# JasonHopeSpace/panda

Measured on AMD Instinct MI355X. Metric: MSM points/s (BN254, 2^24), higher is better.
Workload: dtype u32; 1 GPU; BN254 MSM 2^24 points per GPU, Jacobian output, bases and scalars resident in HBM; curve=bn254, log_points_per_gpu=24, exchange=none

## Files before the change

panda_amd/csrc/fe29.h:

```cpp
#pragma once
#include <stdint.h>

#include "fe29_params.h"

#if defined(__HIPCC__)
#define PANDA_HD __host__ __device__ inline __attribute__((always_inline))
#else
#define PANDA_HD inline __attribute__((always_inline))
#endif

#if defined(FE29_CHECK)
#include <assert.h>
#define FE29_SHADOW_DECL unsigned __int128 shadow = 0;
#define FE29_SHADOW_MAC(x, y) shadow += (unsigned __int128)(x) * (y);
#define FE29_SHADOW_SHIFT()                                      \
    assert(shadow < ((unsigned __int128)1 << 64) && "fe29 column accumulator overflow"); \
    shadow >>= 29;
#else
#define FE29_SHADOW_DECL
#define FE29_SHADOW_MAC(x, y)
#define FE29_SHADOW_SHIFT()
#endif

#if defined(__HIP_DEVICE_COMPILE__) && !defined(FE29_NO_ASM)
// ... 359 lines not shown
    Fe<F> t;
    fe_add_nr(t, a, b);
    fe_norm(r, t);
}

template <class F>
struct SubMargin {
    static constexpr int value = (F::P[F::N - 1] >= 16) ? 1 : 6;
};

template <class F, int KB>
PANDA_HD void fe_sub(Fe<F> &r, const Fe<F> &a, const Fe<F> &b)
{
    if constexpr (IsExt2<F>::value) {
        fe_sub<typename F::Base, KB>(ext_c0(r), ext_c0(a), ext_c0(b));
        fe_sub<typename F::Base, KB>(ext_c1(r), ext_c1(a), ext_c1(b));
        return;
    } else {
    constexpr int K = KB + SubMargin<F>::value;
    static_assert(K <= 200, "subtraction constant table too small");
    Fe<F> t;
#pragma unroll
    for (int i = 0; i < F::N; i++) {
#if defined(FE29_CHECK)
        assert((u64)a.l[i] + F::KP[K][i] >= b.l[i] && (u64)a.l[i] + F::KP[K][i] - b.l[i] < (1ull << 32) && "fe_sub limb range");
#endif
        t.l[i] = a.l[i] + F::KP[K][i] - b.l[i];
    }
    fe_norm(r, t);
    }
}

template <class F, int K>
PANDA_HD constexpr u32 fe_kp30(int i)
{
    return i == 0 ? F::KP[K][0] - (2u << LIMB_BITS) : (i < F::N - 1 ? F::KP[K][i] - (2u << LIMB_BITS) + 2u : F::KP[K][i] + 2u);
}

template <class F>
struct RawOperandOk {
    static constexpr bool value = F::N <= 9;
};

template <class F, int KB>
PANDA_HD void fe_sub_raw(Fe<F> &r, const Fe<F> &a, const Fe<F> &b)
{
    static_assert(RawOperandOk<F>::value, "no column headroom for a raw operand in this field");
    constexpr int K = KB + SubMargin<F>::value;
    static_assert(K <= 200, "subtraction constant table too small");
#pragma unroll
    for (int i = 0; i < F::N; i++) {
        const u32 kp = fe_kp30<F, K>(i);
#if defined(FE29_CHECK)
        assert((u64)a.l[i] + kp >= b.l[i] && (u64)a.l[i] + kp - b.l[i] < (1ull << 31) + (1ull << 24) && "fe_sub_raw limb range");
#endif
        r.l[i] = a.l[i] + kp - b.l[i];
    }
}

template <class F, int K, int U>
PANDA_HD constexpr u32 fe_kp_bias(int i)
{
    static_assert(U >= 2 && U <= 4, "bias in units of 2^29");
    return i == 0 ? F::KP[K][0] - ((u32)(4 - U) << LIMB_BITS) : (i < F::N - 1 ? F::KP[K][i] - ((u32)(4 - U) << LIMB_BITS) + (u32)(4 - U) : F::KP[K][i] + (u32)(4 - U));
}
template <class F, int KB, int U>
PANDA_HD void fe_sub_raw_bias(Fe<F> &r, const Fe<F> &a, const Fe<F> &b)
{
    static_assert(RawOperandOk<F>::value, "no column headroom for a raw operand in this field");
    constexpr int K = KB + SubMargin<F>::value;
    static_assert(K <= 200, "subtraction constant table too small");
#pragma unroll
    for (int i = 0; i < F::N; i++) {
        const u32 kp = fe_kp_bias<F, K, U>(i);
#if defined(FE29_CHECK)
        assert((u64)a.l[i] + kp >= b.l[i] && (u64)a.l[i] + kp - b.l[i] < 3 * (1ull << 30) + 64 && "fe_sub_raw_bias limb range");
#endif
        r.l[i] = a.l[i] + kp - b.l[i];
    }
}

template <class F, int KB>
PANDA_HD void fe_neg_raw(Fe<F> &r, const Fe<F> &a)
{
    static_assert(RawOperandOk<F>::value, "no column headroom for a raw operand in this field");
    constexpr int K = KB + SubMargin<F>::value;
#pragma unroll
    for (int i = 0; i < F::N; i++) {
        const u32 kp = fe_kp30<F, K>(i);
#if defined(FE29_CHECK)
        assert(kp >= a.l[i] && "fe_neg_raw limb range");
#endif
        r.l[i] = kp - a.l[i];
    }
}

template <class F, int KB>
struct SubGrowth {
    static constexpr int value = F::KEFF[KB + SubMargin<F>::value];
};

template <class F, int KB>
PANDA_HD void fe_neg(Fe<F> &r, const Fe<F> &a)
{
    if constexpr (IsExt2<F>::value) {
        fe_neg<typename F::Base, KB>(ext_c0(r), ext_c0(a));
        fe_neg<typename F::Base, KB>(ext_c1(r), ext_c1(a));
        return;
    } else {
    constexpr int K = KB + SubMargin<F>::value;
    Fe<F> t;
#pragma unroll
    for (int i = 0; i < F::N; i++) {
#if defined(FE29_CHECK)
        assert(F::KP[K][i] >= a.l[i] && "fe_neg limb range");
#endif
        t.l[i] = F::KP[K][i] - a.l[i];
    }
    fe_norm(r, t);
    }
}

template <class F>
PANDA_HD void fe_unpack(Fe<F> &r, const u32 *w)
{
    constexpr int N = F::N, L = F::L;
#pragma unroll
    for (int k = 0; k < N; k++) {
        const int bit = 29 * k, wi = bit >> 5, sh = bit & 31;
        u32 v = 0;
        if (wi < L) {
            v = w[wi] >> sh;
            if (sh > 3 && wi + 1 < L) v |= w[wi + 1] << (32 - sh);
        }
        r.l[k] = (k < N - 1) ? (v & LIMB_MASK) : v;
    }
}

template <class F>
PANDA_HD void fe_pack(u32 *w, const Fe<F> &a)
{
    constexpr int N = F::N, L = F::L;
#pragma unroll
    for (int i = 0; i < L; i++) {
        const int bit = 32 * i, j = bit / 29, s = bit - 29 * j;
        u32 v = a.l[j] >> s;
        if (j + 1 < N) v |= a.l[j + 1] << (29 - s);
        if (29 - s + 29 < 32 && j + 2 < N) v |= a.l[j + 2] << (58 - s);
        w[i] = v;
    }
}

template <class F>
PANDA_HD void fe_carry(Fe<F> &a)
{
#pragma unroll
    for (int i = 0; i < F::N - 1; i++) {
#if defined(FE29_CHECK)
        assert((u64)a.l[i + 1] + (a.l[i] >> LIMB_BITS) < (1ull << 32) && "fe_carry limb range");
#endif
        a.l[i + 1] += a.l[i] >> LIMB_BITS;
        a.l[i] &= LIMB_MASK;
    }
}

template <class F>
PANDA_HD void fe_reduce_once(Fe<F> &a)
{
    constexpr int N = F::N;
    u32 d[N];
    u32 borrow = 0;
#pragma unroll
    for (int i = 0; i < N; i++) {
        u32 t = a.l[i] - F::P[i] - borrow;
        borrow = t >> 31;
        d[i] = (i < N - 1) ? (t & LIMB_MASK) : t;
    }
#pragma unroll
    for (int i = 0; i < N; i++) a.l[i] = borrow ? a.l[i] : d[i];
}

template <class F>
PANDA_HD void fe_reduce_small_2p(Fe<F> &a)
{
    constexpr int N = F::N;
    fe_carry(a);
    u32 m;
    if constexpr (F::P[N - 1] >= (1u << 16)) {
        constexpr u64 C = (1ull << 52) / ((u64)F::P[N - 1] + 1);
        m = (u32)(((u64)a.l[N - 1] * C) >> 52);
    } else {
        constexpr u64 D = ((u64)F::P[N - 1] << LIMB_BITS) + F::P[N - 2] + 1;
        static_assert(F::P[N - 1] < (1u << 12) && D >= (1u << 16), "fe_reduce_small: two-limb quotient estimate needs 2^16 <= D, top limb of p < 2^12");
        constexpr u64 C = (1ull << 52) / D;
        const u64 T = ((u64)a.l[N - 1] << LIMB_BITS) | a.l[N - 2];
        m = (u32)((T * C) >> 52);
    }
    int64_t carry = 0;
#pragma unroll
    for (int i = 0; i < N; i++) {
        int64_t t = (int64_t)a.l[i] - (int64_t)((u64)m * F::P[i]) + carry;
        a.l[i] = (i < N - 1) ? ((u32)t & LIMB_MASK) : (u32)t;
        carry = t >> LIMB_BITS;
    }
}

template <class F>
PANDA_HD void fe_reduce_small(Fe<F> &a)
{
    fe_reduce_small_2p(a);
    fe_reduce_once(a);
}

template <class F>
struct FeTw {
    u32 w[F::N];
    u32 q[F::N];
};

#if defined(FE29_DEVICE_CHAINS)
template <class F, bool UNIFORM, int C>
__device__ inline __attribute__((always_inline)) void fe29_shoup_hi_col(uint64_t &acc, const uint32_t *x, const uint32_t *wq, uint32_t *q)
{
    constexpr int N = F::N;
    constexpr int I0 = C < N ? 0 : C - N + 1;
    constexpr int CNT = (C < N ? C : N - 1) - I0 + 1;
    if constexpr (C == N - 2) {
        if constexpr (UNIFORM)
            MacChain<CNT>::vs0(acc, x + I0, wq + (C - I0));
        else
            MacChain<CNT>::vv0(acc, x + I0, wq + (C - I0));
    } else if constexpr (UNIFORM)
        MacChain<CNT>::vs(acc, x + I0, wq + (C - I0));
    else
        MacChain<CNT>::vv(acc, x + I0, wq + (C - I0));
    if constexpr (C >= N) q[C - N] = (uint32_t)acc & ((1u << 29) - 1);
    acc >>= 29;
}
template <class F, bool UNIFORM, int... C>
__device__ inline __attribute__((always_inline)) void fe29_shoup_hi_cols(uint64_t &acc, const uint32_t *x, const uint32_t *wq, uint32_t *q, std::integer_sequence<int, C...>)
{
    (fe29_shoup_hi_col<F, UNIFORM, F::N - 2 + C>(acc, x, wq, q), ...);
}
template <class F, bool UNIFORM, int C>
__device__ inline __attribute__((always_inline)) void fe29_shoup_lo_col(uint64_t &acc, const uint32_t *x, const uint32_t *w, const uint32_t *q, uint32_t *out)
{
    if constexpr (C == 0) {
        if constexpr (UNIFORM)
            MacChain<1>::vs0(acc, x, w);
        else
            MacChain<1>::vv0(acc, x, w);
    } else if constexpr (UNIFORM)
        MacChain<C + 1>::vs(acc, x, w + C);
    else
        MacChain<C + 1>::vv(acc, x, w + C);
    MacChain<C + 1>::vs(acc, q, &F::PNEG[C]);
    out[C] = (uint32_t)acc & ((1u << 29) - 1);
    if constexpr (C + 1 < F::N) acc >>= 29;
}
template <class F, bool UNIFORM, int... C>
__device__ inline __attribute__((always_inline)) void fe29_shoup_lo_cols(uint64_t &acc, const uint32_t *x, const uint32_t *w, const uint32_t *q, uint32_t *out,
                                                                         std::integer_sequence<int, C...>)
{
    (fe29_shoup_lo_col<F, UNIFORM, C>(acc, x, w, q, out), ...);
}
template <class F, bool UNIFORM, int... C>
__device__ inline __attribute__((always_inline)) void fe29_shoup_hi_cols_x2(uint64_t &a0, uint64_t &a1, const uint32_t *x0, const uint32_t *x1, const uint32_t *wq0,
                                                                            const uint32_t *wq1, uint32_t *q0, uint32_t *q1, std::integer_sequence<int, C...>)
{
    ((fe29_shoup_hi_col<F, UNIFORM, F::N - 2 + C>(a0, x0, wq0, q0), fe29_shoup_hi_col<F, UNIFORM, F::N - 2 + C>(a1, x1, wq1, q1)), ...);
}
template <class F, bool UNIFORM, int... C>
__device__ inline __attribute__((always_inline)) void fe29_shoup_lo_cols_x2(uint64_t &a0, uint64_t &a1, const uint32_t *x0, const uint32_t *x1, const uint32_t *w0,
                                                                            const uint32_t *w1, const uint32_t *q0, const uint32_t *q1, uint32_t *o0, uint32_t *o1,
                                                                            std::integer_sequence<int, C...>)
{
    ((fe29_shoup_lo_col<F, UNIFORM, C>(a0, x0, w0, q0, o0), fe29_shoup_lo_col<F, UNIFORM, C>(a1, x1, w1, q1, o1)), ...);
}
#endif

template <class F, bool UNIFORM = false>
PANDA_HD void fe_mul_shoup(Fe<F> &r, const Fe<F> &x, const u32 *w, const u32 *wq)
{
    constexpr int N = F::N;
    static_assert(RawOperandOk<F>::value, "no column headroom for a raw operand in this field");
    u32 q[N], out[N];
    u64 acc = 0;
#if defined(FE29_DEVICE_CHAINS)
    fe29_shoup_hi_cols<F, UNIFORM>(acc, x.l, wq, q, std::make_integer_sequence<int, N + 1>());
    q[N - 1] = (u32)acc & LIMB_MASK;
    acc = 0;
    fe29_shoup_lo_cols<F, UNIFORM>(acc, x.l, w, q, out, std::make_integer_sequence<int, N>());
#pragma unroll
    for (int i = 0; i < N; i++) r.l[i] = out[i];
    return;
#endif
    {
        FE29_SHADOW_DECL
#pragma unroll
        for (int c = N - 2; c <= 2 * N - 2; c++) {
#pragma unroll
            for (int i = (c < N ? 0 : c - N + 1); i <= (c < N ? c : N - 1); i++) {
#if defined(FE29_CHECK)
                assert(x.l[i] < 3 * (1ull << 30) + 64 && wq[c - i] < (1u << 29) && "fe_mul_shoup operand range");
#endif
                FE29_MAC(acc, x.l[i], wq[c - i]);
// ... 218 lines not shown
```

panda_amd/csrc/msm_impl.h:

```cpp
#pragma once
#include <algorithm>
#include <vector>

#include "curve29_quad.h"
#include "msm_sort.h"
#include "panda_internal.h"

namespace panda {

struct MsmRegistration {
    const void *wire;
    void *converted;
    unsigned log_n, curve;
    int device;
    bool tabled;
    WindowPlan plan;
    size_t bytes;
    const uint32_t *samples;
    uint64_t hash;
};
hipError_t msm_hash_wire(const void *d_buf, size_t bytes, hipStream_t s, uint64_t *hash);

struct MsmTuning {
    unsigned window_bits;
// ... 152 lines not shown
        uint4 v = s4[i];
        dst[4 * i] = v.x;
        dst[4 * i + 1] = v.y;
        dst[4 * i + 2] = v.z;
        dst[4 * i + 3] = v.w;
    }
}

template <int WORDS>
__device__ __forceinline__ void load_words_stream(u32 *dst, const u32 *src)
{
    static_assert(WORDS % 4 == 0, "vector loads");
    typedef u32 v4u __attribute__((ext_vector_type(4)));
    const v4u *s4 = reinterpret_cast<const v4u *>(src);
#pragma unroll
    for (int i = 0; i < WORDS / 4; i++) {
        const v4u v = __builtin_nontemporal_load(&s4[i]);
        dst[4 * i] = v.x;
        dst[4 * i + 1] = v.y;
        dst[4 * i + 2] = v.z;
        dst[4 * i + 3] = v.w;
    }
}

template <int WORDS>
__device__ __forceinline__ void store_words(u32 *dst, const u32 *src)
{
    uint4 *d4 = reinterpret_cast<uint4 *>(dst);
#pragma unroll
    for (int i = 0; i < WORDS / 4; i++) d4[i] = make_uint4(src[4 * i], src[4 * i + 1], src[4 * i + 2], src[4 * i + 3]);
}


template <class F>
__global__ void __launch_bounds__(256) k_convert_bases(const u32 *__restrict__ wire, u32 *__restrict__ out, u64 n)
{
    constexpr int L = F::L;
    u64 i = (u64)blockIdx.x * blockDim.x + threadIdx.x;
    if (i >= n) return;
    u32 w[2 * L], o[2 * L];
    load_words<2 * L>(w, wire + i * 2 * L);
    Fe<F> x, y;
    bool inf = affine_from_wire(x, y, w);
    fe_reduce_once(x);
    fe_reduce_once(y);
    fe_pack(o, x);
    fe_pack(o + L, y);
    if (inf) {
#pragma unroll
        for (int k = 0; k < 2 * L; k++) o[k] = 0;
    }
    store_words<2 * L>(out + i * 2 * L, o);
}

template <class F>
__device__ __noinline__ void xyzz_add_outlined(Xyzz<F> &acc, const Xyzz<F> &q)
{
    xyzz_add(acc, q);
}
template <class F>
__device__ __noinline__ void xyzz_dbl_outlined(Xyzz<F> &r, const Xyzz<F> &p)
{
    xyzz_dbl(r, p);
}
template <class F>
__device__ __forceinline__ void xyzz_add_k(Xyzz<F> &acc, const Xyzz<F> &q)
{
    if constexpr (IsExt2<F>::value)
        xyzz_add_outlined(acc, q);
    else
        xyzz_add(acc, q);
}
template <class F>
__device__ __forceinline__ void xyzz_dbl_k(Xyzz<F> &r, const Xyzz<F> &p)
{
    if constexpr (IsExt2<F>::value)
        xyzz_dbl_outlined(r, p);
    else
        xyzz_dbl(r, p);
}

template <class F>
__device__ __noinline__ void xyzz_add_quad_outlined(Xyzz<F> &acc, const Xyzz<F> &q, unsigned role)
{
    xyzz_add_quad(acc, q, role);
}
template <class F>
__device__ __noinline__ void xyzz_dbl_quad_outlined(Xyzz<F> &r, const Xyzz<F> &p, unsigned role)
{
    xyzz_dbl_quad(r, p, role);
}
template <class F>
__device__ __forceinline__ void xyzz_add_q(Xyzz<F> &acc, const Xyzz<F> &q, unsigned role)
{
    if constexpr (IsExt2<F>::value)
        xyzz_add_quad_outlined(acc, q, role);
    else
        xyzz_add_quad(acc, q, role);
}
template <class F>
__device__ __forceinline__ void xyzz_dbl_q(Xyzz<F> &r, const Xyzz<F> &p, unsigned role)
{
    if constexpr (IsExt2<F>::value)
        xyzz_dbl_quad_outlined(r, p, role);
    else
        xyzz_dbl_quad(r, p, role);
}

__global__ void __launch_bounds__(panda::REG_SAMPLES * 16) k_take_samples(const u32 *__restrict__ wire, u32 *__restrict__ samples, u64 n, unsigned row_words)
{
    const unsigned t = threadIdx.x >> 4, l = threadIdx.x & 15;
    const u64 row = panda::sample_row(t, n);
    for (unsigned k = l; k < row_words; k += 16) samples[t * row_words + k] = wire[row * row_words + k];
}

__device__ __forceinline__ u32 owner_bucket(const u32 *off, u32 NB, u32 pos)
{
    u32 lo = 0, hi = NB;
    while (hi - lo > 1) {
        u32 mid = (lo + hi) >> 1;
        if (off[mid] <= pos) lo = mid;
        else hi = mid;
    }
    return lo;
}

__global__ void __launch_bounds__(256) k_chunk_first(const u32 *__restrict__ off, u32 *__restrict__ first, unsigned NB, unsigned K, unsigned chunks)
{
    const unsigned w = blockIdx.y;
    const u32 *ow = off + (u64)w * (NB + 1);
    u32 *fw = first + (u64)w * chunks;
    const unsigned b = blockIdx.x * blockDim.x + threadIdx.x;
    u32 t0 = 0, t1 = 0;
    if (b < NB) {
        const u32 lo = ow[b], hi = ow[b + 1];
        t0 = (lo + K - 1) / K;
        t1 = min((u32)((hi + K - 1) / K), (u32)chunks);
    }
    const unsigned lane = threadIdx.x & 63u;
    u64 wide = __ballot(t1 > t0 + 4);
    while (wide) {
        const int src = __ffsll((long long)wide) - 1;
        wide &= wide - 1;
        const u32 a = (u32)__shfl((int)t0, src), e = (u32)__shfl((int)t1, src), owner = (u32)__shfl((int)b, src);
        for (u32 t = a + lane; t < e; t += 64) fw[t] = owner;
    }
    if (t1 <= t0 + 4)
        for (u32 t = t0; t < t1; t++) fw[t] = b;
}

#ifndef PANDA_ROW_MASK
#define PANDA_ROW_MASK 0x7fffffffu
#endif
template <class F>
struct PackedBase {
    u32 w[2 * F::L];
};

template <class F>
__device__ __forceinline__ void fetch_base(PackedBase<F> &b, const u32 *bases, u32 entry)
{
#if defined(PANDA_ROWS_NT)
    load_words_stream<2 * F::L>(b.w, bases + (u64)(entry & PANDA_ROW_MASK) * 2 * F::L);
#else
    load_words<2 * F::L>(b.w, bases + (u64)(entry & PANDA_ROW_MASK) * 2 * F::L);
#endif
}

template <class F, bool RAW = false>
__device__ __forceinline__ void unpack_base(Fe<F> &x, Fe<F> &y, bool &inf, const PackedBase<F> &b, u32 entry)
{
    constexpr int L = F::L;
    u32 nz = 0;
#pragma unroll
    for (int k = 0; k < 2 * L; k++) nz |= b.w[k];
    inf = (nz == 0);
    fe_unpack(x, b.w);
    fe_unpack(y, b.w + L);
    if (entry >> 31) {
        Fe<F> ny;
        if constexpr (RAW)
            fe_neg_raw<F, 1>(ny, y);
        else
            fe_neg<F, 1>(ny, y);
        y = ny;
    }
}

#ifndef ACC_RAW_Y
#define ACC_RAW_Y false
#endif
struct AccPart {
    const u32 *pos;
    unsigned lo, hi, last, hi_bucket;
    u32 *queue;
};

template <class F>
__device__ __forceinline__ void fetch_base_lds(uint4 *lds_wave, const u32 *bases, u32 entry)
{
    const u32 *src = bases + (u64)(entry & PANDA_ROW_MASK) * 2 * F::L;
#pragma unroll
    for (int j = 0; j < 2 * F::L / 4; j++)
        __builtin_amdgcn_global_load_lds((const __attribute__((address_space(1))) void *)(src + 4 * j), (__attribute__((address_space(3))) void *)(lds_wave + j * 64), 16, 0, 0);
}
template <class F>
__device__ __forceinline__ void read_base_lds(PackedBase<F> &b, const uint4 *lds_wave, unsigned lane)
{
    asm volatile("s_waitcnt vmcnt(0)" ::: "memory");
#pragma unroll
    for (int j = 0; j < 2 * F::L / 4; j++) {
        const uint4 v = lds_wave[j * 64 + lane];
        b.w[4 * j] = v.x;
        b.w[4 * j + 1] = v.y;
        b.w[4 * j + 2] = v.z;
        b.w[4 * j + 3] = v.w;
    }
}

template <class F, bool LDSROW, bool SWLDS = false>
__device__ __forceinline__ void accumulate_chunk(const u32 *__restrict__ bases, const u32 *__restrict__ sw, const u32 *__restrict__ ow, u32 *__restrict__ bw, u32 *__restrict__ pw,
                                                 u32 b, u32 start, u32 end, uint4 *lds_wave, unsigned lane, uint4 *lds_words = nullptr)
{
    constexpr int PW = 4 * F::N;
    u32 next = ow[b + 1];
    bool run_starts_inside = ow[b] >= start;
    Xyzz<F> acc;
    xyzz_set_identity(acc);

    PackedBase<F> next_base;
    const bool quads = ((reinterpret_cast<uintptr_t>(sw + start) & 15) == 0);
    const bool sectors = SWLDS && ((reinterpret_cast<uintptr_t>(sw + start) & 63) == 0);
    auto sector_to_lds = [&](u32 sector) {
        const u32 *src = sw + start + 16 * sector;
#pragma unroll
        for (int q = 0; q < 4; q++)
            __builtin_amdgcn_global_load_lds((const __attribute__((address_space(1))) void *)(src + 4 * q),
                                             (__attribute__((address_space(3))) void *)(lds_words + (sector & 1u) * 256 + q * 64), 16, 0, 0);
    };
    uint4 quad = make_uint4(0, 0, 0, 0);
    if constexpr (SWLDS) {
        if (sectors) {
            sector_to_lds(0);
            if (start + 16 < end) sector_to_lds(1);
            asm volatile("s_waitcnt vmcnt(0)" ::: "memory");
            quad = lds_words[lane];
        } else if (quads)
            quad = *reinterpret_cast<const uint4 *>(sw + start);
    } else if (quads)
        quad = *reinterpret_cast<const uint4 *>(sw + start);
    u32 cur_entry = quads ? quad.x : sw[start];
    u32 ahead_entry = quads ? quad.y : (start + 1 < end ? sw[start + 1] : 0u);
    if constexpr (LDSROW)
        fetch_base_lds<F>(lds_wave, bases, cur_entry);
    else
        fetch_base<F>(next_base, bases, cur_entry);
    for (u32 pos = start; pos < end; pos++) {
        Fe<F> cx, cy;
        bool cinf;
        const u32 entry = cur_entry;
        if constexpr (LDSROW) read_base_lds<F>(next_base, lds_wave, lane);
        unpack_base<F, ACC_RAW_Y && RawOperandOk<F>::value>(cx, cy, cinf, next_base, entry);
        const bool boundary = pos >= next;
        if (boundary) {
            store_xyzz<F>(run_starts_inside ? bw + (u64)b * PW : pw, acc);
            run_starts_inside = true;
            do {
                b++;
                next = ow[b + 1];
            } while (next <= pos);
            if (cinf)
                xyzz_set_identity(acc);
            else {
                Fe<F> ty;
                fe_norm(ty, cy);
                xyzz_from_affine(acc, cx, ty);
            }
        }
        if (pos + 1 < end) {
            cur_entry = ahead_entry;
            if constexpr (LDSROW)
                fetch_base_lds<F>(lds_wave, bases, cur_entry);
            else
                fetch_base<F>(next_base, bases, cur_entry);
            if (pos + 2 < end) {
                if (quads) {
                    const u32 idx = pos + 2 - start;
                    if ((idx & 3u) == 0) {
                        if (SWLDS && sectors) {
                            if ((idx & 15u) == 0 && start + idx + 16 < end) sector_to_lds((idx >> 4) + 1);
                            quad = lds_words[((idx >> 4) & 1u) * 256 + ((idx >> 2) & 3u) * 64 + lane];
                        } else
                            quad = *reinterpret_cast<const uint4 *>(sw + pos + 2);
                    }
                    ahead_entry = (idx & 2u) ? ((idx & 1u) ? quad.w : quad.z) : ((idx & 1u) ? quad.y : quad.x);
                } else
                    ahead_entry = sw[pos + 2];
            }
        }
        if (boundary) continue;
        if (cinf) continue;
        if (xyzz_is_identity(acc)) {
            Fe<F> ty;
            fe_norm(ty, cy);
            xyzz_from_affine(acc, cx, ty);
            continue;
        }
        const int rare = xyzz_madd_core(acc, cx, cy);
        if (rare) {
            if (rare == 1) {
                PackedBase<F> again;
                fetch_base<F>(again, bases, entry);
                unpack_base<F>(cx, cy, cinf, again, entry);
                xyzz_dbl_affine(acc, cx, cy);
            } else
                xyzz_set_identity(acc);
        }
    }
    const bool starts_inside = run_starts_inside;
    const bool ends_inside = next <= end;
    u32 *dst = (starts_inside && ends_inside) ? bw + (u64)b * PW : (starts_inside ? pw + PW : pw);
    store_xyzz<F>(dst, acc);
}

template <class F, bool PERSIST, int WAVES = AccWaves<F>::value, bool LDSROW = false, bool SWLDS = false>
__global__ void __launch_bounds__(128, WAVES) k_accumulate(const u32 *__restrict__ bases, const u32 *__restrict__ sorted, const u32 *__restrict__ off,
                                                    u32 *__restrict__ bucket_acc, u32 *__restrict__ parts, u64 stride, unsigned NB, unsigned K,
                                                    unsigned chunks, u32 *__restrict__ long_count, const u32 *__restrict__ stale, AccPart part,
                                                    const u32 *__restrict__ chunk_first)
{
    constexpr int PW = 4 * F::N;
    const unsigned w = blockIdx.y;
    const unsigned t0 = blockIdx.x * blockDim.x + threadIdx.x;
    const u32 *fw = chunk_first ? chunk_first + (u64)w * chunks : nullptr;
    if (t0 == 0) long_count[w] = 0;
    if (stale && *stale) return;
    const u32 *ow = off + (u64)w * (NB + 1);
    const u32 lo_pos = part.pos ? part.pos[part.lo] : 0u;
    const u32 limit = part.pos ? part.pos[part.hi] : ow[NB];
    const unsigned search_hi = part.pos ? part.hi_bucket : NB;
    const bool takes_short_chunk = part.pos ? part.last != 0 : true;
    const u32 *sw = sorted + (u64)w * stride;
    u32 *bw = bucket_acc + (u64)w * NB * PW;
    __shared__ uint4 s_rows[LDSROW ? 2 * (2 * F::L / 4) * 64 : 1];
    uint4 *lds_wave = s_rows + (threadIdx.x >> 6) * (LDSROW ? (2 * F::L / 4) * 64 : 0);
    __shared__ uint4 s_words[SWLDS ? 2 * 512 : 1];
    uint4 *lds_words = s_words + (threadIdx.x >> 6) * (SWLDS ? 512 : 0);
    const unsigned lane = threadIdx.x & 63u;
    if constexpr (PERSIST) {
        const unsigned first = lo_pos / K;
#pragma unroll 1
        for (;;) {
            unsigned base = 0;
            if (lane == 0) base = atomicAdd(part.queue, 64u);
            base = __builtin_amdgcn_readfirstlane(base) + first;
            if (base >= chunks || (u64)base * K >= limit) return;
            const unsigned t = base + lane;
            const u32 start = t * K;
            u32 end = start + K;
            bool mine = t < chunks && start < limit;
            bool clamped = false;
            if (end > limit) {
                mine = mine && takes_short_chunk;
                end = limit;
                clamped = true;
            }
            if (mine && (end > lo_pos || clamped))
                accumulate_chunk<F, LDSROW, SWLDS>(bases, sw, ow, bw, parts + ((u64)w * chunks + t) * 2 * PW, fw ? fw[t] : owner_bucket(ow, search_hi, start), start, end, lds_wave, lane, lds_words);
        }
    } else {
        const unsigned t = t0;
        if (t >= chunks) return;
        const u32 start = t * K;
        if (start >= limit) return;
        u32 end = start + K;
        bool clamped = false;
        if (end > limit) {
            if (!takes_short_chunk) return;
            end = limit;
            clamped = true;
        }
        if (end > lo_pos || clamped)
            accumulate_chunk<F, LDSROW, SWLDS>(bases, sw, ow, bw, parts + ((u64)w * chunks + t) * 2 * PW, fw ? fw[t] : owner_bucket(ow, search_hi, start), start, end, lds_wave, lane, lds_words);
    }
}

template <class F>
__device__ __forceinline__ void fetch_rows_shared(uint4 *lds_wave, const u32 *bases, u32 entry, unsigned lane)
{
    constexpr unsigned P = 2 * F::L / 4;
#pragma unroll
    for (unsigned m = 0; m < P; m++) {
        const unsigned f = m * 64 + lane;
        const u32 e = (u32)__shfl((int)entry, (int)(f / P));
        const u32 *src = bases + (u64)(e & PANDA_ROW_MASK) * 2 * F::L + 4 * (f % P);
        __builtin_amdgcn_global_load_lds((const __attribute__((address_space(1))) void *)src, (__attribute__((address_space(3))) void *)(lds_wave + m * 64), 16, 0, 0);
    }
}
template <class F>
__device__ __forceinline__ void read_row_shared(PackedBase<F> &b, const uint4 *lds_wave, unsigned lane)
{
    constexpr unsigned P = 2 * F::L / 4;
    asm volatile("s_waitcnt vmcnt(0)" ::: "memory");
#pragma unroll
    for (unsigned j = 0; j < P; j++) {
        const uint4 v = lds_wave[lane * P + j];
        b.w[4 * j] = v.x;
        b.w[4 * j + 1] = v.y;
        b.w[4 * j + 2] = v.z;
        b.w[4 * j + 3] = v.w;
    }
}

template <class F, int WAVES = AccWaves<F>::value>
__global__ void __launch_bounds__(128, WAVES) k_accumulate_shared(const u32 *__restrict__ bases, const u32 *__restrict__ sorted, const u32 *__restrict__ off,
                                                           u32 *__restrict__ bucket_acc, u32 *__restrict__ parts, u64 stride, unsigned NB, unsigned K,
                                                           unsigned chunks, u32 *__restrict__ long_count, const u32 *__restrict__ stale)
{
    constexpr int PW = 4 * F::N;
    constexpr unsigned P = 2 * F::L / 4;
    const unsigned w = blockIdx.y;
    const unsigned t = blockIdx.x * blockDim.x + threadIdx.x;
    if (t == 0) long_count[w] = 0;
    if (stale && *stale) return;
    const u32 *ow = off + (u64)w * (NB + 1);
    const u32 *sw = sorted + (u64)w * stride;
    u32 *bw = bucket_acc + (u64)w * NB * PW;
    u32 *pw = parts + ((u64)w * chunks + t) * 2 * PW;
    const u32 limit = ow[NB];
    const bool has = t < chunks && (u64)t * K < limit;
    if (__ballot(has) == 0) return;
    const u32 start = has ? t * K : 0u;
    const u32 end = has ? (u32)min((u64)start + K, (u64)limit) : 0u;
    __shared__ uint4 s_rows[2 * P * 64];
    uint4 *lds_wave = s_rows + (threadIdx.x >> 6) * (P * 64);
    const unsigned lane = threadIdx.x & 63u;

    u32 b = 0, next = 0;
    bool run_starts_inside = false;
    if (has) {
        b = owner_bucket(ow, NB, start);
        next = ow[b + 1];
        run_starts_inside = ow[b] >= start;
    }
    Xyzz<F> acc;
    xyzz_set_identity(acc);
    const bool quads = has && ((reinterpret_cast<uintptr_t>(sw + start) & 15) == 0);
    uint4 quad = make_uint4(0, 0, 0, 0);
    if (quads) quad = *reinterpret_cast<const uint4 *>(sw + start);
    u32 cur_entry = has ? (quads ? quad.x : sw[start]) : 0u;
    u32 ahead_entry = quads ? quad.y : (start + 1 < end ? sw[start + 1] : 0u);
    fetch_rows_shared<F>(lds_wave, bases, cur_entry, lane);
#pragma unroll 1
    for (u32 i = 0; i < K; i++) {
        const u32 pos = start + i;
        const bool live = pos < end;
        const u32 entry = cur_entry;
        PackedBase<F> row;
        read_row_shared<F>(row, lds_wave, lane);
        Fe<F> cx, cy;
        bool cinf;
        unpack_base<F, ACC_RAW_Y && RawOperandOk<F>::value>(cx, cy, cinf, row, entry);
        const bool boundary = live && pos >= next;
        if (boundary) {
            store_xyzz<F>(run_starts_inside ? bw + (u64)b * PW : pw, acc);
            run_starts_inside = true;
            do {
                b++;
                next = ow[b + 1];
            } while (next <= pos);
            if (cinf)
                xyzz_set_identity(acc);
            else {
                Fe<F> ty;
// ... 854 lines not shown
```

Measured before the change: 995.2 million points/s.

## Slim the bucket accumulate loop with vector row loads, packed-word negation and identity flag

Reworks the per-point accumulate loop in several ways. Base rows are loaded as 128-bit vector tuples. The y negation is done on packed words before unpacking. Only y words are tested for infinity. An explicit identity flag replaces the per-iteration identity check, and a boundary path reuses the madd/identity logic instead of duplicating affine conversion. The scalar-quad index now shifts instead of being selected, and the LDS sector prefetch uses finer vmcnt waits. The aim is fewer VALU ops and registers per iteration in the hot loop, at the cost of extra compiler barriers and more complex control flow.

```diff
diff --git a/panda_amd/csrc/fe29.h b/panda_amd/csrc/fe29.h
--- a/panda_amd/csrc/fe29.h
+++ b/panda_amd/csrc/fe29.h
@@ -535,6 +535,26 @@
 }
 
 template <class F>
+PANDA_HD void fe_words_neg(u32 *r, const u32 *w)
+{
+    static_assert(!IsExt2<F>::value, "prime fields only");
+#if defined(__clang__)
+    unsigned borrow = 0;
+#pragma unroll
+    for (int i = 0; i < F::L; i++) r[i] = __builtin_subc(F::PW[i], w[i], borrow, &borrow);
+#else
+    u32 borrow = 0;
+#pragma unroll
+    for (int i = 0; i < F::L; i++) {
+        const u32 d = F::PW[i] - w[i];
+        const u32 out = (u32)(F::PW[i] < w[i]) | (u32)(d < borrow);
+        r[i] = d - borrow;
+        borrow = out;
+    }
+#endif
+}
+
+template <class F>
 PANDA_HD void fe_carry(Fe<F> &a)
 {
 #pragma unroll
diff --git a/panda_amd/csrc/msm_impl.h b/panda_amd/csrc/msm_impl.h
--- a/panda_amd/csrc/msm_impl.h
+++ b/panda_amd/csrc/msm_impl.h
@@ -328,6 +328,24 @@
 #ifndef PANDA_ROW_MASK
 #define PANDA_ROW_MASK 0x7fffffffu
 #endif
+#ifndef PANDA_ACC_ITEMS
+#define PANDA_ACC_ITEMS 0x3fu
+#endif
+constexpr unsigned ACC_ITEM_ROW_TUPLES = 32u;
+constexpr unsigned ACC_ITEM_WORDS_NEG = 1u;
+constexpr unsigned ACC_ITEM_Y_IDENTITY = 2u;
+constexpr unsigned ACC_ITEM_QUAD_SHIFT = 4u;
+constexpr unsigned ACC_ITEM_ID_FLAG = 8u;
+constexpr unsigned ACC_ITEM_BOUNDARY = 16u;
+template <class F>
+struct AccSlim {
+    static constexpr bool value = !IsExt2<F>::value && F::N <= 9;
+};
+template <class F>
+__host__ __device__ constexpr bool acc_item(unsigned item)
+{
+    return AccSlim<F>::value && (PANDA_ACC_ITEMS & item) != 0;
+}
 template <class F>
 struct PackedBase {
     u32 w[2 * F::L];
@@ -343,23 +361,65 @@
 #endif
 }
 
-template <class F, bool RAW = false>
+template <class F>
+struct PackedRow {
+    typedef u32 v4u __attribute__((ext_vector_type(4)));
+    v4u q[2 * F::L / 4];
+};
+template <class F>
+__device__ __forceinline__ void fetch_row(PackedRow<F> &r, const u32 *bases, u32 entry)
+{
+    typedef typename PackedRow<F>::v4u v4u;
+    const v4u *s4 = reinterpret_cast<const v4u *>(bases + (u64)(entry & PANDA_ROW_MASK) * 2 * F::L);
+#pragma unroll
+    for (int j = 0; j < 2 * F::L / 4; j++) {
+#if defined(PANDA_ROWS_NT)
+        r.q[j] = __builtin_nontemporal_load(&s4[j]);
+#else
+        r.q[j] = s4[j];
+#endif
+    }
+}
+template <class F>
+__device__ __forceinline__ void row_words(PackedBase<F> &b, const PackedRow<F> &r)
+{
+#pragma unroll
+    for (int j = 0; j < 2 * F::L / 4; j++) {
+        b.w[4 * j] = r.q[j].x;
+        b.w[4 * j + 1] = r.q[j].y;
+        b.w[4 * j + 2] = r.q[j].z;
+        b.w[4 * j + 3] = r.q[j].w;
+    }
+}
+
+template <class F, bool RAW = false, bool SLIM = false>
 __device__ __forceinline__ void unpack_base(Fe<F> &x, Fe<F> &y, bool &inf, const PackedBase<F> &b, u32 entry)
 {
     constexpr int L = F::L;
+    constexpr bool WORDS_NEG = SLIM && acc_item<F>(ACC_ITEM_WORDS_NEG);
+    constexpr int NZ_FROM = SLIM && acc_item<F>(ACC_ITEM_Y_IDENTITY) ? L : 0;
     u32 nz = 0;
 #pragma unroll
-    for (int k = 0; k < 2 * L; k++) nz |= b.w[k];
+    for (int k = NZ_FROM; k < 2 * L; k++) nz |= b.w[k];
+    if constexpr (WORDS_NEG) asm volatile("" : "+v"(nz));
     inf = (nz == 0);
     fe_unpack(x, b.w);
-    fe_unpack(y, b.w + L);
-    if (entry >> 31) {
-        Fe<F> ny;
-        if constexpr (RAW)
-            fe_neg_raw<F, 1>(ny, y);
-        else
-            fe_neg<F, 1>(ny, y);
-        y = ny;
+    if constexpr (WORDS_NEG) {
+        u32 yw[L];
+#pragma unroll
+        for (int k = 0; k < L; k++) yw[k] = b.w[L + k];
+        if (entry >> 31) fe_words_neg<F>(yw, b.w + L);
+        fe_unpack(y, yw);
+    } else {
+        fe_unpack(y, b.w + L);
+        if (entry >> 31) {
+            Fe<F> ny;
+            if constexpr (RAW)
+                fe_neg_raw<F, 1>(ny, y);
+            else
+                fe_neg<F, 1>(ny, y);
+            y = ny;
+        }
     }
 }
 
@@ -407,18 +467,18 @@
     PackedBase<F> next_base;
     const bool quads = ((reinterpret_cast<uintptr_t>(sw + start) & 15) == 0);
     const bool sectors = SWLDS && ((reinterpret_cast<uintptr_t>(sw + start) & 63) == 0);
-    auto sector_to_lds = [&](u32 sector) {
-        const u32 *src = sw + start + 16 * sector;
+    auto sector_to_lds = [&](u32 sector, const u32 *src) {
+        const u32 buffer = (u32)__builtin_amdgcn_readfirstlane((int)(sector & 1u));
 #pragma unroll
         for (int q = 0; q < 4; q++)
             __builtin_amdgcn_global_load_lds((const __attribute__((address_space(1))) void *)(src + 4 * q),
-                                             (__attribute__((address_space(3))) void *)(lds_words + (sector & 1u) * 256 + q * 64), 16, 0, 0);
+                                             (__attribute__((address_space(3))) void *)(lds_words + buffer * 256 + q * 64), 16, 0, 0);
     };
     uint4 quad = make_uint4(0, 0, 0, 0);
     if constexpr (SWLDS) {
         if (sectors) {
-            sector_to_lds(0);
-            if (start + 16 < end) sector_to_lds(1);
+            sector_to_lds(0, sw + start);
+            if (start + 16 < end) sector_to_lds(1, sw + start + 16);
             asm volatile("s_waitcnt vmcnt(0)" ::: "memory");
             quad = lds_words[lane];
         } else if (quads)
@@ -427,75 +487,145 @@
         quad = *reinterpret_cast<const uint4 *>(sw + start);
     u32 cur_entry = quads ? quad.x : sw[start];
     u32 ahead_entry = quads ? quad.y : (start + 1 < end ? sw[start + 1] : 0u);
+    constexpr bool ROW_TUPLES = !LDSROW && acc_item<F>(ACC_ITEM_ROW_TUPLES);
+    constexpr int ROW_LOADS = 2 * F::L / 4;
+    PackedRow<F> next_row;
     if constexpr (LDSROW)
         fetch_base_lds<F>(lds_wave, bases, cur_entry);
+    else if constexpr (ROW_TUPLES)
+        fetch_row<F>(next_row, bases, cur_entry);
     else
         fetch_base<F>(next_base, bases, cur_entry);
-    for (u32 pos = start; pos < end; pos++) {
+    constexpr bool QUAD_SHIFT = acc_item<F>(ACC_ITEM_QUAD_SHIFT);
+    constexpr bool ID_FLAG = acc_item<F>(ACC_ITEM_ID_FLAG);
+    constexpr bool SLIM_BOUNDARY = ID_FLAG && acc_item<F>(ACC_ITEM_BOUNDARY);
+    constexpr bool Y_STORABLE = acc_item<F>(ACC_ITEM_WORDS_NEG) || !(ACC_RAW_Y && RawOperandOk<F>::value);
+    bool acc_id = true;
+    u32 *brun = bw + (u64)b * PW;
+    if constexpr (QUAD_SHIFT) {
+        quad.x = quad.y;
+        quad.y = quad.z;
+        quad.z = quad.w;
+    }
+    u32 trip = 0;
+    for (u32 pos = start; pos < end; pos++, trip++) {
         Fe<F> cx, cy;
         bool cinf;
         const u32 entry = cur_entry;
         if constexpr (LDSROW) read_base_lds<F>(next_base, lds_wave, lane);
-        unpack_base<F, ACC_RAW_Y && RawOperandOk<F>::value>(cx, cy, cinf, next_base, entry);
+        if constexpr (ROW_TUPLES) row_words<F>(next_base, next_row);
+        unpack_base<F, ACC_RAW_Y && RawOperandOk<F>::value, true>(cx, cy, cinf, next_base, entry);
+        if constexpr (ROW_TUPLES) {
+#pragma unroll
+            for (int i = 0; i < F::N; i++) asm volatile("" : "+v"(cx.l[i]), "+v"(cy.l[i]));
+        }
         const bool boundary = pos >= next;
         if (boundary) {
-            store_xyzz<F>(run_starts_inside ? bw + (u64)b * PW : pw, acc);
-            run_starts_inside = true;
-            do {
-                b++;
-                next = ow[b + 1];
-            } while (next <= pos);
-            if (cinf)
-                xyzz_set_identity(acc);
-            else {
+            if constexpr (SLIM_BOUNDARY) {
+                store_xyzz<F>(run_starts_inside ? brun : pw, acc);
+                run_starts_inside = true;
+                do {
+                    b++;
+                    brun += PW;
+                    next = ow[b + 1];
+                } while (next <= pos);
+                if (cinf) xyzz_set_identity(acc);
+                acc_id = true;
+            } else {
+                store_xyzz<F>(run_starts_inside ? bw + (u64)b * PW : pw, acc);
+                run_starts_inside = true;
+                do {
+                    b++;
+                    next = ow[b + 1];
+                } while (next <= pos);
+                acc_id = cinf;
+                if (cinf)
+                    xyzz_set_identity(acc);
+                else {
+                    Fe<F> ty;
+                    fe_norm(ty, cy);
+                    xyzz_from_affine(acc, cx, ty);
+                }
+            }
+        }
+        if (pos + 1 < end) {
+            cur_entry = ahead_entry;
+            if constexpr (LDSROW)
+                fetch_base_lds<F>(lds_wave, bases, cur_entry);
+            else if constexpr (ROW_TUPLES)
+                fetch_row<F>(next_row, bases, cur_entry);
+            else
+                fetch_base<F>(next_base, bases, cur_entry);
+            if (pos + 2 < end) {
+                if (quads) {
+                    const u32 idx = QUAD_SHIFT ? trip + 2 : pos + 2 - start;
+                    if ((idx & 3u) == 0) {
+                        if (SWLDS && sectors) {
+                            if ((idx & 15u) == 0) {
+                                if (pos + 18 < end) {
+                                    sector_to_lds((idx >> 4) + 1, sw + pos + 18);
+                                    asm volatile("s_waitcnt vmcnt(%0)" ::"n"(ROW_LOADS + 4) : "memory");
+                                } else
+                                    asm volatile("s_waitcnt vmcnt(%0)" ::"n"(ROW_LOADS) : "memory");
+                            }
+                            quad = lds_words[((idx >> 4) & 1u) * 256 + ((idx >> 2) & 3u) * 64 + lane];
+                        } else {
+                            quad = *reinterpret_cast<const uint4 *>(sw + pos + 2);
+                            if constexpr (ROW_TUPLES) asm volatile("" : "+v"(quad.x), "+v"(quad.y), "+v"(quad.z), "+v"(quad.w));
+                        }
+                    } else if constexpr (QUAD_SHIFT) {
+                        quad.x = quad.y;
+                        quad.y = quad.z;
+                        quad.z = quad.w;
+                    }
+                    if constexpr (QUAD_SHIFT)
+                        ahead_entry = quad.x;
+                    else
+                        ahead_entry = (idx & 2u) ? ((idx & 1u) ? quad.w : quad.z) : ((idx & 1u) ? quad.y : quad.x);
+                } else {
+                    ahead_entry = sw[pos + 2];
+                    if constexpr (ROW_TUPLES) asm volatile("" : "+v"(ahead_entry));
+                }
+            }
+        }
+        if constexpr (!SLIM_BOUNDARY)
+            if (boundary) continue;
+        if (cinf) continue;
+        if (ID_FLAG ? acc_id : xyzz_is_identity(acc)) {
+            if constexpr (SLIM_BOUNDARY && Y_STORABLE) {
+#pragma unroll
+                for (int i = 0; i < F::N; i++) {
+                    asm("v_mov_b32 %0, %1" : "=v"(acc.X.l[i]) : "v"(cx.l[i]));
+                    asm("v_mov_b32 %0, %1" : "=v"(acc.Y.l[i]) : "v"(cy.l[i]));
+                }
+                fe_one(acc.ZZ);
+                fe_one(acc.ZZZ);
+            } else {
                 Fe<F> ty;
                 fe_norm(ty, cy);
                 xyzz_from_affine(acc, cx, ty);
             }
-        }
-        if (pos + 1 < end) {
-            cur_entry = ahead_entry;
-            if constexpr (LDSROW)
-                fetch_base_lds<F>(lds_wave, bases, cur_entry);
-            else
-                fetch_base<F>(next_base, bases, cur_entry);
-            if (pos + 2 < end) {
-                if (quads) {
-                    const u32 idx = pos + 2 - start;
-                    if ((idx & 3u) == 0) {
-                        if (SWLDS && sectors) {
-                            if ((idx & 15u) == 0 && start + idx + 16 < end) sector_to_lds((idx >> 4) + 1);
-                            quad = lds_words[((idx >> 4) & 1u) * 256 + ((idx >> 2) & 3u) * 64 + lane];
-                        } else
-                            quad = *reinterpret_cast<const uint4 *>(sw + pos + 2);
-                    }
-                    ahead_entry = (idx & 2u) ? ((idx & 1u) ? quad.w : quad.z) : ((idx & 1u) ? quad.y : quad.x);
-                } else
-                    ahead_entry = sw[pos + 2];
-            }
-        }
-        if (boundary) continue;
-        if (cinf) continue;
-        if (xyzz_is_identity(acc)) {
-            Fe<F> ty;
-            fe_norm(ty, cy);
-            xyzz_from_affine(acc, cx, ty);
+            acc_id = false;
             continue;
         }
         const int rare = xyzz_madd_core(acc, cx, cy);
         if (rare) {
             if (rare == 1) {
                 PackedBase<F> again;
-                fetch_base<F>(again, bases, entry);
-                unpack_base<F>(cx, cy, cinf, again, entry);
+                const u32 same = acc_item<F>(ACC_ITEM_WORDS_NEG) ? sw[pos] : entry;
+                fetch_base<F>(again, bases, same);
+                unpack_base<F, false, true>(cx, cy, cinf, again, same);
                 xyzz_dbl_affine(acc, cx, cy);
-            } else
+                acc_id = xyzz_is_identity(acc);
+            } else {
                 xyzz_set_identity(acc);
+                acc_id = true;
+            }
         }
     }
     const bool starts_inside = run_starts_inside;
     const bool ends_inside = next <= end;
-    u32 *dst = (starts_inside && ends_inside) ? bw + (u64)b * PW : (starts_inside ? pw + PW : pw);
+    u32 *dst = (starts_inside && ends_inside) ? (SLIM_BOUNDARY ? brun : bw + (u64)b * PW) : (starts_inside ? pw + PW : pw);
     store_xyzz<F>(dst, acc);
 }
 
```

After: 1.012 billion points/s (median of 6 runs). 1.7% higher.
